# Sudaraka88/LDWeaver

Measured on AMD Instinct MI355X. Metric: MI SNP-pairs/sec, higher is better.
Workload: dtype i8

## Files before the change

### ldweaver_amd/csrc/ldw_apx.hip

```cpp
#include <algorithm>
#include <cmath>
#include <cstdlib>
#include <cstring>

#include "ldw_apx.h"
#include "ldw_dev.h"

using namespace ldw;

namespace ldw {

namespace {
constexpr int64_t APX_PROD_CAP = 12000;
struct ProdTable {
    std::vector<int32_t> val;
    std::vector<uint8_t> a, b;
    ProdTable() {
        std::vector<std::pair<int32_t, std::pair<uint8_t, uint8_t>>> all;
        for (int x = 0; x <= 127; ++x)
            for (int y = x; y <= 127; ++y) all.push_back({x * y, {(uint8_t)x, (uint8_t)y}});
        std::sort(all.begin(), all.end());
        for (auto &e : all)
            if (val.empty() || val.back() != e.first) {
                val.push_back(e.first);
// ... 824 lines not shown
    else if (tile == 33 && !P.fuse) {
        const int ntx = (P.RFpad + 95) / 96, nty = (P.RTpad + 95) / 96;
        if (P.fine) hipLaunchKernelGGL((gemm_apx_kernel<3, 3, true, 2>), dim3((unsigned)((ntx + 1) / 2), (unsigned)((nty + 1) / 2)), dim3(256), lds, st, P);
        else hipLaunchKernelGGL((gemm_apx_kernel<3, 3, false, 2>), dim3((unsigned)((ntx + 1) / 2), (unsigned)((nty + 1) / 2)), dim3(256), lds, st, P);
    }
    else if (tile == 224 && !P.fuse) {
        const int ntx = P.RFpad / 64, nty = P.RTpad / 64;
        if (P.fine) hipLaunchKernelGGL((gemm_apx_kernel<2, 2, true, 4>), dim3((unsigned)((ntx + 1) / 2), (unsigned)((nty + 1) / 2)), dim3(256), lds, st, P);
        else hipLaunchKernelGGL((gemm_apx_kernel<2, 2, false, 4>), dim3((unsigned)((ntx + 1) / 2), (unsigned)((nty + 1) / 2)), dim3(256), lds, st, P);
    }
    else if (tile == 24 && !P.fuse) LDW_APX_LAUNCH(2, 4)
    else if (tile == 32 && !P.fuse) {
        const int ntx = P.RFpad / 64, nty = (P.RTpad + 95) / 96;
        if (P.fine) hipLaunchKernelGGL((gemm_apx_kernel<3, 2, true, 3>), dim3((unsigned)((ntx + 1) / 2), (unsigned)((nty + 1) / 2)), dim3(256), lds, st, P);
        else hipLaunchKernelGGL((gemm_apx_kernel<3, 2, false, 3>), dim3((unsigned)((ntx + 1) / 2), (unsigned)((nty + 1) / 2)), dim3(256), lds, st, P);
    }
#endif
    else LDW_APX_LAUNCH(4, 2)
#undef LDW_APX_LAUNCH
    LDW_HIP(hipGetLastError());
    {
        const int tl = P.fuse ? 42 : tile;
        const int MTv = (P.fuse && P.skip_ctr) ? APX_MT : (tl == 22 || tl == 24 || tl == 224 ? 2 : (tl == 32 || tl == 33 ? 3 : 4)), NTv = tl == 24 ? 4 : (tl == 33 ? 3 : 2), TH = 32 * MTv, TWd = 32 * NTv;
        int64_t waves = 0;
        for (int ty = 0; ty * TH < P.RTpad; ++ty) {
            const int ntx = P.RFpad / TWd;
            if (!P.lower_only) waves += ntx;
            else for (int tx = 0; tx < ntx; ++tx) waves += (tx * TWd + TWd - 1 < ty * TH) ? 0 : 1;
        }
        c->gemm_stat[0] += 1;
        if (P.fuse) c->gemm_stat[5] += 1;
        c->gemm_stat[1] += 2.0 * (double)waves * TH * TWd * ((double)P.M2 * 128.0);
        if (P.fuse && P.skip_ctr) {
            c->apx_ops_per_wave = 2.0 * TH * TWd * ((double)P.M2 * 128.0);
            c->apx_waves_total += waves;
        }
    }
    return LDW_OK;
}

struct PairArgs {
    const uint64_t *Mbits;
    int64_t KW;
    int nwords, path, nseg;
    int seg_in_lds;
    const PopSeg *segs;
    const int32_t *wbeg, *row0;
    int32_t zero_row;
    int64_t *sums;
    EpiArgs A;
    unsigned long long *ghist;
};

template <int CA, int CB>
__device__ __forceinline__ void pair_sums_body(const PairArgs &P, int path, const int32_t *s_wbeg, const PopSeg *s_segs) {
    constexpr bool GENB = CA == 4 && CB == 4;
    const EpiArgs &A = P.A;
    const int sub = path * PAIR_SHARDS + (int)blockIdx.y;
    unsigned int n = A.pl_n[sub];
    n = n > A.pl_cap ? A.pl_cap : n;
    const int lane = threadIdx.x & 63;
    const PairEnt *list = A.pl_pairs + (int64_t)sub * A.pl_cap;
    constexpr int KW = 3, KS = 2;
    uint32_t smask[KW][KS];
    int64_t sV[KW][KS];
    bool more[KW];
#pragma unroll
    for (int k = 0; k < KW; ++k) {
        const int w = lane + 64 * k;
        int s0 = 0, s1 = 0;
        if (w < P.nwords) {
            s0 = s_wbeg[w] & 0x7FFFFFFF;
            s1 = s_wbeg[w + 1] & 0x7FFFFFFF;
        }
        more[k] = s1 - s0 > KS;
#pragma unroll
        for (int q = 0; q < KS; ++q) {
            const bool on = s0 + q < s1 && !more[k];
            smask[k][q] = on ? s_segs[s0 + q].mask : 0u;
            sV[k][q] = on ? s_segs[s0 + q].V : 0;
        }
    }
    for (unsigned int idx = blockIdx.x * 4u + (threadIdx.x >> 6); idx < n; idx += gridDim.x * 4u) {
        const PairEnt e = list[idx];
        const uint32_t era = (uint32_t)__builtin_amdgcn_readfirstlane((int)e.ra), erb = (uint32_t)__builtin_amdgcn_readfirstlane((int)e.rb);
        const int r0a = (int)(era & 0x1FFFFFFFu), na = (int)(era >> 29), r0b = (int)(erb & 0x1FFFFFFFu), nb = (int)(erb >> 29);
        const uint32_t *fr[CA], *tr[CB];
#pragma unroll
        for (int i = 0; i < CA; ++i) fr[i] = reinterpret_cast<const uint32_t *>(P.Mbits + (int64_t)(i < na ? r0a + i : P.zero_row) * P.KW);
#pragma unroll
        for (int j = 0; j < CB; ++j) tr[j] = reinterpret_cast<const uint32_t *>(P.Mbits + (int64_t)(j < nb ? r0b + j : P.zero_row) * P.KW);
        int64_t s[CB][CA];
#pragma unroll
        for (int j = 0; j < CB; ++j)
#pragma unroll
            for (int i = 0; i < CA; ++i) s[j][i] = 0;
        uint32_t f[KW][CA], tt[KW][CB];
#pragma unroll
        for (int k = 0; k < KW; ++k) {
            const int w = lane + 64 * k;
            const bool in = w < P.nwords;
#pragma unroll
            for (int i = 0; i < CA; ++i) f[k][i] = (in && (!GENB || i < na)) ? fr[i][w] : 0u;
#pragma unroll
            for (int j = 0; j < CB; ++j) tt[k][j] = (in && (!GENB || j < nb)) ? tr[j][w] : 0u;
        }
// ... 5 lines not shown
                for (int sg = s0; sg < s1; ++sg) {
                    const PopSeg seg = s_segs[sg];
#pragma unroll
                    for (int j = 0; j < CB; ++j)
#pragma unroll
                        for (int i = 0; i < CA; ++i)
                            if (!GENB || (i < na && j < nb)) s[j][i] += (int64_t)((uint64_t)__popc(f[k][i] & tt[k][j] & seg.mask) * (uint64_t)seg.V);
                }
            } else {
#pragma unroll
                for (int q2 = 0; q2 < KS; ++q2)
#pragma unroll
                    for (int j = 0; j < CB; ++j)
#pragma unroll
                        for (int i = 0; i < CA; ++i)
                            if (!GENB || (i < na && j < nb)) s[j][i] += (int64_t)((uint64_t)__popc(f[k][i] & tt[k][j] & smask[k][q2]) * (uint64_t)sV[k][q2]);
            }
        }
        for (int w = lane + 64 * KW; w < P.nwords; w += 64) {
            uint32_t f2[CA], t2[CB];
#pragma unroll
            for (int i = 0; i < CA; ++i) f2[i] = (!GENB || i < na) ? fr[i][w] : 0u;
#pragma unroll
            for (int j = 0; j < CB; ++j) t2[j] = (!GENB || j < nb) ? tr[j][w] : 0u;
            const int s0 = s_wbeg[w] & 0x7FFFFFFF, s1 = s_wbeg[w + 1] & 0x7FFFFFFF;
            for (int sg = s0; sg < s1; ++sg) {
                const PopSeg seg = s_segs[sg];
#pragma unroll
                for (int j = 0; j < CB; ++j)
#pragma unroll
                    for (int i = 0; i < CA; ++i)
                        if (!GENB || (i < na && j < nb)) s[j][i] += (int64_t)((uint64_t)__popc(f2[i] & t2[j] & seg.mask) * (uint64_t)seg.V);
            }
        }
#pragma unroll
        for (int j = 0; j < CB; ++j)
#pragma unroll
            for (int i = 0; i < CA; ++i) {
                int64_t v = s[j][i];
                if (!GENB || (i < na && j < nb)) {
#pragma unroll
                    for (int off = 32; off > 0; off >>= 1) v += __shfl_xor(v, off);
                }
                if (lane == 0) P.sums[((int64_t)sub * A.pl_cap + idx) * 16 + j * 4 + i] = v;
            }
    }
}

template <bool GEN>
__global__ __launch_bounds__(256) void k_pair_sums(PairArgs P) {
    extern __shared__ __attribute__((aligned(16))) uint8_t pop_smem[];
    int32_t *s_wbeg = reinterpret_cast<int32_t *>(pop_smem);
    PopSeg *s_segs = reinterpret_cast<PopSeg *>(pop_smem + (((size_t)P.nwords + 4) * 4 + 15) / 16 * 16);
    const int path = GEN ? 4 : (int)blockIdx.z;
    if (blockIdx.x * 4u >= P.A.pl_n[path * PAIR_SHARDS + (int)blockIdx.y]) return;
    if (P.seg_in_lds) {
        for (int i = threadIdx.x; i < P.nwords + 1; i += 256) s_wbeg[i] = P.wbeg[i];
        for (int i = threadIdx.x; i < P.nseg; i += 256) s_segs[i] = P.segs[i];
        __syncthreads();
    } else {
        s_wbeg = const_cast<int32_t *>(P.wbeg);
        s_segs = const_cast<PopSeg *>(P.segs);
    }
    if constexpr (GEN) {
        pair_sums_body<4, 4>(P, 4, s_wbeg, s_segs);
    } else {
        switch (path) {
            case 0: pair_sums_body<1, 1>(P, 0, s_wbeg, s_segs); break;
            case 1: pair_sums_body<2, 1>(P, 1, s_wbeg, s_segs); break;
            case 2: pair_sums_body<1, 2>(P, 2, s_wbeg, s_segs); break;
            default: pair_sums_body<2, 2>(P, 3, s_wbeg, s_segs); break;
        }
    }
}

template <int CA, int CB>
__device__ __forceinline__ void pair_sums_bits_body(const PairArgs &P, int path, const int64_t *sVT, int stride) {
    constexpr bool GENB = CA == 4 && CB == 4;
    const EpiArgs &A = P.A;
    const int sub = path * PAIR_SHARDS + (int)blockIdx.y;
    unsigned int n = A.pl_n[sub];
    n = n > A.pl_cap ? A.pl_cap : n;
    const int lane = threadIdx.x & 63;
    const PairEnt *list = A.pl_pairs + (int64_t)sub * A.pl_cap;
    for (unsigned int idx = blockIdx.x * 4u + (threadIdx.x >> 6); idx < n; idx += gridDim.x * 4u) {
        const PairEnt e = list[idx];
        const uint32_t era = (uint32_t)__builtin_amdgcn_readfirstlane((int)e.ra), erb = (uint32_t)__builtin_amdgcn_readfirstlane((int)e.rb);
        const int r0a = (int)(era & 0x1FFFFFFFu), na = (int)(era >> 29), r0b = (int)(erb & 0x1FFFFFFFu), nb = (int)(erb >> 29);
        const uint32_t *fr[CA], *tr[CB];
#pragma unroll
        for (int i = 0; i < CA; ++i) fr[i] = reinterpret_cast<const uint32_t *>(P.Mbits + (int64_t)(i < na ? r0a + i : P.zero_row) * P.KW);
#pragma unroll
        for (int j = 0; j < CB; ++j) tr[j] = reinterpret_cast<const uint32_t *>(P.Mbits + (int64_t)(j < nb ? r0b + j : P.zero_row) * P.KW);
        int64_t s[CB][CA];
#pragma unroll
        for (int j = 0; j < CB; ++j)
#pragma unroll
            for (int i = 0; i < CA; ++i) s[j][i] = 0;
        for (int w = lane; w < P.nwords; w += 64) {
            uint32_t f[CA], t[CB], uf = 0u, ut = 0u;
#pragma unroll
            for (int i = 0; i < CA; ++i) {
                f[i] = (!GENB || i < na) ? fr[i][w] : 0u;
                uf |= f[i];
            }
#pragma unroll
            for (int j = 0; j < CB; ++j) {
// ... 2 lines not shown
            }
            uint32_t u = uf & ut;
            while (u) {
                const int b = __builtin_ctz(u);
                u &= u - 1u;
                const int64_t v = sVT[b * stride + w];
#pragma unroll
                for (int j = 0; j < CB; ++j)
#pragma unroll
                    for (int i = 0; i < CA; ++i)
                        if (CA * CB == 1 || (((f[i] & t[j]) >> b) & 1u)) s[j][i] += v;
            }
        }
#pragma unroll
        for (int j = 0; j < CB; ++j)
#pragma unroll
            for (int i = 0; i < CA; ++i) {
                int64_t v = s[j][i];
                if (!GENB || (i < na && j < nb)) {
#pragma unroll
                    for (int off = 32; off > 0; off >>= 1) v += __shfl_xor(v, off);
                }
                if (lane == 0) P.sums[((int64_t)sub * A.pl_cap + idx) * 16 + j * 4 + i] = v;
            }
    }
}

template <bool GEN>
__global__ __launch_bounds__(256) void k_pair_sums_bits(PairArgs P, const int64_t *__restrict__ vpos, int stride) {
    extern __shared__ __attribute__((aligned(16))) uint8_t pop_smem[];
    int64_t *sVT = reinterpret_cast<int64_t *>(pop_smem);
    const int path = GEN ? 4 : (int)blockIdx.z;
    if (blockIdx.x * 4u >= P.A.pl_n[path * PAIR_SHARDS + (int)blockIdx.y]) return;
    for (int i = threadIdx.x; i < 32 * stride; i += 256) {
        const int b = i / stride, w = i - b * stride;
        sVT[i] = w < P.nwords ? vpos[32 * w + b] : 0;
    }
    __syncthreads();
    if constexpr (GEN) {
        pair_sums_bits_body<4, 4>(P, 4, sVT, stride);
    } else {
        switch (path) {
            case 0: pair_sums_bits_body<1, 1>(P, 0, sVT, stride); break;
            case 1: pair_sums_bits_body<2, 1>(P, 1, sVT, stride); break;
            case 2: pair_sums_bits_body<1, 2>(P, 2, sVT, stride); break;
            default: pair_sums_bits_body<2, 2>(P, 3, sVT, stride); break;
        }
    }
}

constexpr int PAIR_HWIN = 128;

template <int NA, int NB>
__device__ __forceinline__ void pair_mi_body(const PairArgs &P, int path, unsigned int *s_hist) {
    constexpr bool GEN = NA == 0;
    const EpiArgs &A = P.A;
    const EmitArgs &E = A.E;
    const int sub = path * PAIR_SHARDS + (int)blockIdx.y;
    unsigned int n = A.pl_n[sub];
    n = n > A.pl_cap ? A.pl_cap : n;
    const bool square = A.nf == A.nt;
    const PairEnt *list = A.pl_pairs + (int64_t)sub * A.pl_cap;
    const int lane = (int)(threadIdx.x & 63);
    for (unsigned int base = blockIdx.x * 256u + (threadIdx.x & ~63u); base < n; base += gridDim.x * 256u) {
        const unsigned int idx = base + (unsigned int)lane;
        bool valid = idx < n;
        uint32_t t = 0, q = 0;
        if (valid) {
            t = list[idx].t;
            q = list[idx].q;
        }
        const RowPack &RP = A.rowpack[t];
        valid = valid && RP.a_loc >= 0;
        bool cand = false;
        int bk = 0, seg = -1, a_loc = 0, b_loc = 0, sg = 0;
        double mi = 0.0;
        if (valid) {
            const RowSide R = RP.R;
            a_loc = RP.a_loc;
            const ColMeta M = A.colpack[q];
            b_loc = M.bl;
            sg = A.span ? M.ci.pad[0] : 0;
            const int64_t *sp = P.sums + ((int64_t)sub * A.pl_cap + idx) * 16;
            if constexpr (GEN) {
                mi = pair_mi<4, 4>(A, R, M, a_loc, b_loc, square, gacc_plain(sp, 1, 4));
            } else {
                mi = pair_mi_full<NA, NB>(A, R, M, a_loc, b_loc, square, gacc_plain(sp, 1, 4));
            }
            seg = pair_seg(a_loc, b_loc, E.lower_only);
            if (seg >= 0 && E.any_sr && col_is_sr(M.ci, a_loc)) {
                emit_pair_spec(E, M.ci, a_loc, b_loc, R.sa, M.sb, mi, P.ghist);
            } else if (seg >= 0 && E.do_lr && mi >= E.spec_lo) {
                bk = mi_bucket(mi);
                cand = bk >= E.spec_B;
            }
        }
        if (A.span) {
            for (int k = 0; k < A.span; ++k) {
                const bool mine = cand && sg == k;
                const unsigned long long mk = __ballot(mine);
                if (mk == 0ull) continue;
                const int leader = __builtin_ctzll(mk);
                unsigned long long pos = 0;
                if (lane == leader) pos = atomicAdd(A.sseg[k].n_cand, (unsigned long long)__popcll(mk));
                pos = __shfl(pos, leader);
                if (mine) {
                    pos += (unsigned long long)__popcll(mk & ((1ull << lane) - 1ull));
                    A.sseg[k].ckey[pos] = f64_key(mi);
                    A.sseg[k].cval[pos] = ((uint64_t)seg << 62) | ((uint64_t)a_loc + (uint64_t)b_loc * (uint64_t)E.nf);
                    const int w = bk - (E.spec_B > 0 ? E.spec_B : 0);
                    if (w < PAIR_HWIN) atomicAdd(&s_hist[k * PAIR_HWIN + w], 1u);
                    else atomicAdd(&A.sseg[k].ghist[bk], 1ull);
                }
            }
            continue;
        }
        const unsigned long long mk = __ballot(cand);
        if (mk == 0ull) continue;
        const int leader = __builtin_ctzll(mk);
        unsigned long long pos = 0;
        if (lane == leader) pos = atomicAdd(E.n_cand, (unsigned long long)__popcll(mk));
        pos = __shfl(pos, leader);
        if (cand) {
            pos += (unsigned long long)__popcll(mk & ((1ull << lane) - 1ull));
            E.ckey[pos] = f64_key(mi);
            E.cval[pos] = ((uint64_t)seg << 62) | ((uint64_t)a_loc + (uint64_t)b_loc * (uint64_t)E.nf);
            const int w = bk - (E.spec_B > 0 ? E.spec_B : 0);
            if (w < PAIR_HWIN) atomicAdd(&s_hist[w], 1u);
            else atomicAdd(&P.ghist[bk], 1ull);
        }
    }
}

__global__ __launch_bounds__(256) void k_pair_mi(PairArgs P) {
    __shared__ unsigned int s_hist[LDW_SPAN_MAX * PAIR_HWIN];
    for (int i = threadIdx.x; i < LDW_SPAN_MAX * PAIR_HWIN; i += 256) s_hist[i] = 0u;
    __syncthreads();
    switch (blockIdx.z) {
        case 0: pair_mi_body<1, 1>(P, 0, s_hist); break;
        case 1: pair_mi_body<2, 1>(P, 1, s_hist); break;
        case 2: pair_mi_body<1, 2>(P, 2, s_hist); break;
        case 3: pair_mi_body<2, 2>(P, 3, s_hist); break;
        default: pair_mi_body<0, 0>(P, 4, s_hist); break;
    }
    __syncthreads();
    const int hb0 = P.A.E.spec_B > 0 ? P.A.E.spec_B : 0;
    if (P.A.span) {
        for (int i = threadIdx.x; i < P.A.span * PAIR_HWIN; i += 256) {
            const int k = i / PAIR_HWIN, w = i - k * PAIR_HWIN;
            if (s_hist[i] != 0u && hb0 + w < NBINS) atomicAdd(&P.A.sseg[k].ghist[hb0 + w], (unsigned long long)s_hist[i]);
        }
        return;
    }
    if (threadIdx.x < PAIR_HWIN && s_hist[threadIdx.x] != 0u && hb0 + (int)threadIdx.x < NBINS)
        atomicAdd(&P.ghist[hb0 + threadIdx.x], (unsigned long long)s_hist[threadIdx.x]);
}

int launch_pairs_exact(ldw_ctx *c, const EpiArgs &A, unsigned long long *ghist, int64_t *sums, hipStream_t st) {
    PairArgs P;
    memset(&P, 0, sizeof(P));
    P.Mbits = c->Mbits.as<uint64_t>();
    P.KW = c->KW;
    P.nwords = (int)(c->KW * 2);
    P.nseg = c->n_pop_segs;
    P.segs = c->pop_segs.as<PopSeg>();
    P.wbeg = c->pop_wbeg.as<int32_t>();
    P.row0 = c->row0.as<int32_t>();
    P.zero_row = (int32_t)c->R;
    P.sums = sums;
    P.A = A;
    P.ghist = ghist;
    size_t lds = (((size_t)P.nwords + 4) * 4 + 15) / 16 * 16 + (size_t)P.nseg * sizeof(PopSeg);
    P.seg_in_lds = lds <= 60000 ? 1 : 0;
    if (!P.seg_in_lds) lds = 0;
    const int stride = (P.nwords + 31) / 32 * 32;
    const size_t lds_bits = (size_t)32 * stride * 8;
    const bool bits_off = getenv("LDW_NO_PAIR_BITS") != nullptr;
    const bool many_classes = !P.seg_in_lds || P.nseg >= 8 * P.nwords;
    if (many_classes && !bits_off && lds_bits <= 160 * 1024 && c->pop_vpos.p) {
        if (lds_bits > 64 * 1024 && !c->pair_bits_attr) {
            LDW_HIP(hipFuncSetAttribute(reinterpret_cast<const void *>(k_pair_sums_bits<false>), hipFuncAttributeMaxDynamicSharedMemorySize, 160 * 1024));
            LDW_HIP(hipFuncSetAttribute(reinterpret_cast<const void *>(k_pair_sums_bits<true>), hipFuncAttributeMaxDynamicSharedMemorySize, 160 * 1024));
            c->pair_bits_attr = true;
        }
        hipLaunchKernelGGL(k_pair_sums_bits<false>, dim3(256, PAIR_SHARDS, 4), dim3(256), lds_bits, st, P, c->pop_vpos.as<int64_t>(), stride);
        hipLaunchKernelGGL(k_pair_sums_bits<true>, dim3(256, PAIR_SHARDS, 1), dim3(256), lds_bits, st, P, c->pop_vpos.as<int64_t>(), stride);
    } else {
        static const unsigned gx_env = [] { const char *e = getenv("LDW_PAIR_GRID"); return e ? (unsigned)atoi(e) : 0u; }();
        hipLaunchKernelGGL(k_pair_sums<false>, dim3(gx_env ? gx_env : 512u, PAIR_SHARDS, 4), dim3(256), lds, st, P);
        hipLaunchKernelGGL(k_pair_sums<true>, dim3(gx_env ? gx_env : 1024u, PAIR_SHARDS, 1), dim3(256), lds, st, P);
    }
    hipLaunchKernelGGL(k_pair_mi, dim3(64, PAIR_SHARDS, PAIR_PATHS), dim3(256), 0, st, P);
    LDW_HIP(hipGetLastError());
    return LDW_OK;
}

}

namespace ldw {
void warm_apx() {
    hipFuncAttributes a;
    (void)hipFuncGetAttributes(&a, reinterpret_cast<const void *>(&k_pack_panel));
    (void)hipGetLastError();
}
}
```

### ldweaver_amd/csrc/ldw_internal.h

```cpp
#pragma once
#include <hip/hip_runtime.h>
#include <stdint.h>
#include <stdlib.h>
#include <string>
#include <atomic>
#include <memory>
#include <mutex>
#include <thread>
#include <vector>

#include "../../include/ldweaver_amd.h"

#define LDW_NSLOT 3

#ifdef LDW_EXPERIMENTS
#define LDW_HAS_EXPERIMENTS 1
#else
#define LDW_HAS_EXPERIMENTS 0
#endif

namespace ldw {

inline const char *exp_env(const char *name) {
#ifdef LDW_EXPERIMENTS
// ... 40 lines not shown
};
struct BlockTrace {
    int diag = 0, guess = -1, B_true = -1, margin = 0, path = 0 , missed = 0, probed = 0;
    long long n_cand = 0;
};

}

struct ldw_ctx {
    int device = 0;
    hipStream_t stream = nullptr;
    bool own_stream = true;
    hipEvent_t ev[6] = {nullptr, nullptr, nullptr, nullptr, nullptr, nullptr};
    double last_ms[4] = {0, 0, 0, 0};
    int engine = LDW_ENGINE_MFMA;

    int64_t L = 0, N = 0, Npad = 0;
    int64_t KW = 0;
    ldw::DevBuf states;
    ldw::DevBuf chars;
    int64_t cN = 0, cL = 0;
    void *fasta = nullptr;

    bool have_weights = false;
    int nlimbs = 5;
    int frac_bits = 0;
    double neff = 0;
    int64_t total_fixed = 0;
    ldw::DevBuf digits;
    ldw::DevBuf vfixed;
    std::vector<int64_t> h_vfixed;
    std::vector<int64_t> h_vfixed_hi;
    int64_t total_fixed_hi = 0;
    double lo_abs_sum = 0;
    int mixed = 1;

    std::vector<int32_t> h_seq_perm;
    ldw::DevBuf seq_perm;
    int path_mode = 0;
    int select_mode = 0;
    bool apx_ok = false;
    bool apx_fine = false;
    std::string apx_gate = "weights not set";
    ldw::DevBuf dig_a, dig_b;
    ldw::DevBuf apx_shift;
    int apx_e_last = 0;
    int apx_transitions = 0;
    double apx_lost_units = 0;
    double apx_delta = 0;
    std::vector<int64_t> h_vapx;
    ldw::DevBuf slot_papx;
    ldw::DevBuf pop_segs, pop_wbeg;
    ldw::DevBuf pop_vpos;
    bool pair_bits_attr = false;
    int n_pop_segs = 0, n_classes = 0;
    ldw::DevBuf panel[LDW_NSLOT][2];
    ldw::DevBuf Gapx[LDW_NSLOT];
    ldw::DevBuf tab11[2];
    double tab11_lo[2] = {0, 0};
    int tab11_cur[2] = {0, 0};
    int64_t tab11_builds = 0;
    float tab11_c = 0;
    int tab11_nb = 0;
    bool tab11_on = true;
    ldw::DevBuf pair_sums;
    ldw::DevBuf pairs[LDW_NSLOT];
    ldw::DevBuf sub_units[LDW_NSLOT], sub_packs[LDW_NSLOT], sub_bins[LDW_NSLOT], sub_live[LDW_NSLOT];
    ldw::DevBuf scr_live[LDW_NSLOT];
    ldw::DevBuf apx_bins[LDW_NSLOT], apx_clean[LDW_NSLOT];
    ldw::DevBuf apx_mini[LDW_NSLOT];
    ldw::DevBuf apx_units[LDW_NSLOT], apx_packs[LDW_NSLOT];
    int64_t apx_blocks = 0, apx_units_listed = 0, apx_pairs_listed = 0, probe_blocks = 0, generic_blocks = 0;
    bool prune = true;
    ldw::DevBuf apx_skip;
    double apx_ops_per_wave = 0;
    int64_t apx_waves_skipped = 0, apx_waves_total = 0;
    bool span_on = true;
    bool diag_split = false;
    bool span_corners = false;
    int span_max = 8;
    int64_t maybe_entries = 0;
    int64_t pair_list_overflows = 0, maybe_overflows = 0;
    bool maybe_off = false;
    int64_t span_items = 0, span_blocks = 0, span_fallbacks = 0;
    int64_t span_sr_subs = 0;
    bool early_sr = false;
    std::atomic<int64_t> sorted_blocks{0};
    std::mutex order_mtx;
    ldw::DevBuf snp_sup;
    double r_min = 0;
    struct OrderCache { std::vector<int32_t> idx, order; };
    std::vector<std::unique_ptr<OrderCache>> order_cache;

    bool have_meta = false;
    double g = 0;
    ldw::DevBuf r, uqe, POS, paint;
    std::vector<double> h_r;
    std::vector<int32_t> h_POS, h_paint;
    int32_t paint_min = 0, paint_max = 0;
    bool pos_sorted = true;
    double sr_total_dist = -1;
    int64_t sr_total = -1;
    uint64_t sr_share_key = 0;
    int64_t sr_share_rows = -1;

    bool rows_ready = false;
// ... 118 lines not shown
```

### ldweaver_amd/csrc/ldw_mi_items.inc

```
struct HostBlock {
    int64_t nf = 0, nt = 0, n_sr_blk = 0, n_lr_total = 0, blk_no = 0;
    int RFpad = 0, RTpad = 0, slot = 0;
    bool diag = false, fused = false, submitted = false;
    int nf_tiles = 0;
    int gen_t0 = 0, gen_q0 = 0;
    bool mixed = false;
    bool apx = false;
    bool generic = false;
    int guess = -1;
    LoHost lo;
    size_t o_cmax = 0, o_tbase = 0, o_tf = 0, o_band = 0, o_bandl = 0;
    int n_band = -1;
    size_t o_idx_f = 0, o_idx_t = 0, o_rl_f = 0, o_rl_t = 0, o_lrow_f = 0, o_lrow_t = 0, o_perm = 0, o_perm_t = 0, o_cols = 0, o_pos_f = 0,
           o_pos_t = 0, o_cls_f = 0, o_cls_t = 0, total = 0;
    DevPtrs D{};
    EmitArgs E{};
    int spec_B = -1;
    int span = 0;
    int32_t seg_start[LDW_SPAN_MAX] = {}, seg_nt[LDW_SPAN_MAX] = {};
    int64_t seg_lr_total[LDW_SPAN_MAX] = {};
    size_t cand_cap = 0;
    SpanSeg sseg[LDW_SPAN_MAX] = {};
    int pin_slot = -1;
    bool force_plain = false;
// ... 876 lines not shown
    const int32_t *ti = span.span_to.data() + span.seg_start[k];
    LDW_HIP(hipStreamSynchronize(c->stream));
    if (c->gemm_stream) LDW_HIP(hipStreamSynchronize(c->gemm_stream));
    if (int rc = prep_block(c, span.span_from.data(), span.nf, ti, span.seg_nt[k], p, span.slot, span.blk_no + k, hb, nullptr, LDW_NSLOT)) return rc;
    hb.force_plain = force_plain;
    ldw_mi_params q = *p;
    if (force_plain) q.keep_sr = 0;
    hb.sr_base = span.sr_base;
    for (int j = 0; j < k; ++j) hb.sr_base += span.seg_n_sr[j];
    hb.sr_base_fixed = true;
    p = &q;
    if (int rc = submit_a(c, hb, p, sl)) return rc;
    if (int rc = submit_b(c, hb, p, sl)) return rc;
    if (int rc = finish_block(c, hb, p, sl)) return rc;
    LDW_HIP(hipStreamSynchronize(c->stream));
    return LDW_OK;
}

int finish_span(ldw_ctx *c, HostBlock &hb, const ldw_mi_params *p, const SmallLayout &sl) {
    const int s = hb.slot;
    if (hb.span_alone) {
        for (int k = 0; k < hb.span; ++k)
            if (int rc = run_block_alone(c, hb, k, p, sl, false)) return rc;
        LDW_HIP(hipEventRecord(c->ev_done[s], c->stream));
        c->done_recorded[s] = true;
        return LDW_OK;
    }
    LDW_HIP(hipEventSynchronize(c->ev_pick[s]));
    ldw::PickOut picks[LDW_SPAN_MAX];
    for (int k = 0; k < hb.span; ++k) memcpy(&picks[k], static_cast<const char *>(c->pin_pick[s]) + (size_t)k * PICK_STRIDE, sizeof(ldw::PickOut));
    if (c->lrc_recorded) {
        LDW_HIP(hipEventSynchronize(c->ev_lrc));
        memcpy(&c->n_lr, c->pin_lrc, 8);
    }
    const char *d = stage_ptr(c, hb);
    if ((int64_t)c->trace.size() < hb.blk_no + hb.span) c->trace.resize((size_t)(hb.blk_no + hb.span));
    {
        static const bool trace_on = getenv("LDW_BLOCK_TRACE") != nullptr;
        if (trace_on && picks[0].n > 0 && !picks[0].spec_ok) {
            unsigned int pl[PAIR_PATHS * PAIR_SHARDS];
            LDW_HIP(hipMemcpy(pl, c->pairs[s].p, sizeof(pl), hipMemcpyDeviceToHost));
            fprintf(stderr, "[ldw span at block %lld] guess %d, %d segments, pair-list capacity %u, counters by path:", (long long)hb.blk_no, hb.guess, hb.span, pair_cap_for(hb.nf, hb.nt, hb.span));
            for (int pth = 0; pth < PAIR_PATHS; ++pth) {
                unsigned long long tot = 0, mx = 0;
                for (int sh2 = 0; sh2 < PAIR_SHARDS; ++sh2) {
                    tot += pl[pth * PAIR_SHARDS + sh2];
                    mx = std::max<unsigned long long>(mx, pl[pth * PAIR_SHARDS + sh2]);
                }
                fprintf(stderr, "  [%d] total %llu max %llu", pth, tot, mx);
            }
            fprintf(stderr, "\n");
        }
    }
    static const bool sel_fast_on = getenv("LDW_NO_FAST_SELECT") == nullptr && exp_env("LDW_NO_SPAN_SELECT") == nullptr;
    bool batched = sel_fast_on && c->select_mode == 0;
    long long m_max = 0, m_sum = 0;
    for (int k = 0; k < hb.span && batched; ++k) {
        const ldw::PickOut *hp = &picks[k];
        const uint64_t space = (uint64_t)hb.nf * (uint64_t)hb.seg_nt[k];
        const long long n_chunks = (long long)((2 * space + SEL_CHUNK_BITS - 1) / SEL_CHUNK_BITS) + 1, n_super = (n_chunks + SEL_SUPER - 1) / SEL_SUPER;
        batched = !(hp->n > 0 && !hp->spec_ok) && (long long)hp->n_cand <= SEL_MAX && n_super <= SEL_MAX_SUPER && (size_t)hp->n_cand <= hb.cand_cap;
        m_max = std::max<long long>(m_max, (long long)hp->n_cand);
        m_sum += (long long)hp->n_cand;
    }
    if (batched) {
        SelSpan S;
        memset(&S, 0, sizeof(S));
        SpanDoneArgs DA;
        memset(&DA, 0, sizeof(DA));
        S.n = hb.span;
        size_t w_off = 0, c_off = 0;
        size_t woff[LDW_SPAN_MAX], coff[LDW_SPAN_MAX];
        for (int k = 0; k < hb.span; ++k) {
            const uint64_t space = (uint64_t)hb.nf * (uint64_t)hb.seg_nt[k];
            const size_t n_words = (size_t)((2 * space + 31) / 32) + 1, n_chunks = (size_t)((2 * space + SEL_CHUNK_BITS - 1) / SEL_CHUNK_BITS) + 1;
            woff[k] = w_off;
            coff[k] = c_off;
            w_off += (n_words + 63) / 64 * 64;
            c_off += (n_chunks + 63) / 64 * 64;
            S.space[k] = space;
            S.n_super[k] = (int)((n_chunks + SEL_SUPER - 1) / SEL_SUPER);
        }
        if (w_off * 4 > c->sel_bitmap.cap || c_off * 4 > c->sel_chunks.cap || (size_t)LDW_SPAN_MAX * SEL_MAX_SUPER * 4 > c->sel_prefix.cap) {
            if (int rc = c->sel_bitmap.reserve(w_off * 4)) return rc;
            if (int rc = c->sel_chunks.reserve(c_off * 4)) return rc;
            if (int rc = c->sel_prefix.reserve((size_t)LDW_SPAN_MAX * SEL_MAX_SUPER * 4)) return rc;
            LDW_HIP(hipMemsetAsync(c->sel_bitmap.p, 0, c->sel_bitmap.cap, c->stream));
            LDW_HIP(hipMemsetAsync(c->sel_chunks.p, 0, c->sel_chunks.cap, c->stream));
            LDW_HIP(hipMemsetAsync(c->sel_prefix.p, 0, c->sel_prefix.cap, c->stream));
        }
        if (int rc = ensure_links_capacity(c, c->n_sr, c->n_lr + m_sum)) return rc;
        for (int k = 0; k < hb.span; ++k) {
            const ldw::PickOut *hp = &picks[k];
            if (hp->n > 0) update_guess(c, false, hp, false);
            ldw::BlockTrace &tr = c->trace[(size_t)hb.blk_no + k];
            tr = ldw::BlockTrace();
            tr.guess = hb.guess;
            tr.B_true = hp->B_true;
            tr.path = 4;
            tr.n_cand = (long long)hp->n_cand;
            S.ck[k] = hb.sseg[k].ckey;
            S.cv[k] = hb.sseg[k].cval;
            S.pick[k] = reinterpret_cast<ldw::PickOut *>(reinterpret_cast<char *>(sl.pick[s]) + (size_t)k * PICK_STRIDE);
            S.idx_t[k] = reinterpret_cast<const int32_t *>(d + hb.o_idx_t) + hb.seg_start[k];
            S.bitmap[k] = c->sel_bitmap.as<uint32_t>() + woff[k];
            S.chunks[k] = c->sel_chunks.as<uint32_t>() + coff[k];
// ... 127 lines not shown
```

Baseline: 163.1 billion.

## Add opt-in fused exact pair-sum and MI kernels with balanced run scheduling

Adds new kernels that split all pair lists into equal-size runs per wave, reuse loaded bit words across consecutive pairs sharing a row or column, and can fuse the popcount sums with the MI epilogue through LDS instead of global memory. These paths run only when LDW_PAIR_EXACT or LDW_PAIR_RUNS environment variables are set. By default the only behaviour change is that k_pair_sums now processes paths in reverse z order, and a pair-list statistics dump is added behind an env flag. The fused paths raise LDS use and register pressure in exchange for fewer global round trips and better load balance.

```diff
diff --git a/ldweaver_amd/csrc/ldw_apx.hip b/ldweaver_amd/csrc/ldw_apx.hip
--- a/ldweaver_amd/csrc/ldw_apx.hip
+++ b/ldweaver_amd/csrc/ldw_apx.hip
@@ -900,6 +900,149 @@
     unsigned long long *ghist;
 };
 
+constexpr int PAIR_KW = 3, PAIR_KS = 2;
+struct PairSegRegs {
+    uint32_t smask[PAIR_KW][PAIR_KS];
+    int64_t sV[PAIR_KW][PAIR_KS];
+    bool more[PAIR_KW];
+};
+__device__ __forceinline__ void pair_seg_regs(const PairArgs &P, const int32_t *s_wbeg, const PopSeg *s_segs, int lane, PairSegRegs &S) {
+#pragma unroll
+    for (int k = 0; k < PAIR_KW; ++k) {
+        const int w = lane + 64 * k;
+        int s0 = 0, s1 = 0;
+        if (w < P.nwords) {
+            s0 = s_wbeg[w] & 0x7FFFFFFF;
+            s1 = s_wbeg[w + 1] & 0x7FFFFFFF;
+        }
+        S.more[k] = s1 - s0 > PAIR_KS;
+#pragma unroll
+        for (int q = 0; q < PAIR_KS; ++q) {
+            const bool on = s0 + q < s1 && !S.more[k];
+            S.smask[k][q] = on ? s_segs[s0 + q].mask : 0u;
+            S.sV[k][q] = on ? s_segs[s0 + q].V : 0;
+        }
+    }
+}
+template <int CA, int CB>
+struct PairWords {
+    uint32_t f[PAIR_KW][CA], t[PAIR_KW][CB];
+};
+template <int CA, int CB>
+__device__ __forceinline__ const uint32_t *pair_row(const PairArgs &P, int r0, int n, int i) {
+    return reinterpret_cast<const uint32_t *>(P.Mbits + (int64_t)(i < n ? r0 + i : P.zero_row) * P.KW);
+}
+template <int CA, int CB, bool F, bool T>
+__device__ __forceinline__ void pair_load_words(const PairArgs &P, int lane, int r0a, int na, int r0b, int nb, PairWords<CA, CB> &W) {
+    constexpr bool GENB = CA == 4 && CB == 4;
+#pragma unroll
+    for (int k = 0; k < PAIR_KW; ++k) {
+        const int w = lane + 64 * k;
+        const bool in = w < P.nwords;
+        if constexpr (F) {
+#pragma unroll
+            for (int i = 0; i < CA; ++i) W.f[k][i] = (in && (!GENB || i < na)) ? pair_row<CA, CB>(P, r0a, na, i)[w] : 0u;
+        }
+        if constexpr (T) {
+#pragma unroll
+            for (int j = 0; j < CB; ++j) W.t[k][j] = (in && (!GENB || j < nb)) ? pair_row<CA, CB>(P, r0b, nb, j)[w] : 0u;
+        }
+    }
+}
+template <int CA, int CB>
+__device__ __forceinline__ void pair_lane_sums(const PairArgs &P, int lane, int r0a, int na, int r0b, int nb, const PairWords<CA, CB> &W,
+                                               const PairSegRegs &S, const int32_t *s_wbeg, const PopSeg *s_segs, int64_t (&s)[CB][CA]) {
+    constexpr bool GENB = CA == 4 && CB == 4;
+#pragma unroll
+    for (int j = 0; j < CB; ++j)
+#pragma unroll
+        for (int i = 0; i < CA; ++i) s[j][i] = 0;
+#pragma unroll
+    for (int k = 0; k < PAIR_KW; ++k) {
+        if (S.more[k]) {
+            const int w = lane + 64 * k;
+            const int s0 = s_wbeg[w] & 0x7FFFFFFF, s1 = s_wbeg[w + 1] & 0x7FFFFFFF;
+            for (int sg = s0; sg < s1; ++sg) {
+                const PopSeg seg = s_segs[sg];
+#pragma unroll
+                for (int j = 0; j < CB; ++j)
+#pragma unroll
+                    for (int i = 0; i < CA; ++i)
+                        if (!GENB || (i < na && j < nb)) s[j][i] += (int64_t)((uint64_t)__popc(W.f[k][i] & W.t[k][j] & seg.mask) * (uint64_t)seg.V);
+            }
+        } else {
+#pragma unroll
+            for (int q2 = 0; q2 < PAIR_KS; ++q2)
+#pragma unroll
+                for (int j = 0; j < CB; ++j)
+#pragma unroll
+                    for (int i = 0; i < CA; ++i)
+                        if (!GENB || (i < na && j < nb)) s[j][i] += (int64_t)((uint64_t)__popc(W.f[k][i] & W.t[k][j] & S.smask[k][q2]) * (uint64_t)S.sV[k][q2]);
+        }
+    }
+    for (int w = lane + 64 * PAIR_KW; w < P.nwords; w += 64) {
+        uint32_t f2[CA], t2[CB];
+#pragma unroll
+        for (int i = 0; i < CA; ++i) f2[i] = (!GENB || i < na) ? pair_row<CA, CB>(P, r0a, na, i)[w] : 0u;
+#pragma unroll
+        for (int j = 0; j < CB; ++j) t2[j] = (!GENB || j < nb) ? pair_row<CA, CB>(P, r0b, nb, j)[w] : 0u;
+        const int s0 = s_wbeg[w] & 0x7FFFFFFF, s1 = s_wbeg[w + 1] & 0x7FFFFFFF;
+        for (int sg = s0; sg < s1; ++sg) {
+            const PopSeg seg = s_segs[sg];
+#pragma unroll
+            for (int j = 0; j < CB; ++j)
+#pragma unroll
+                for (int i = 0; i < CA; ++i)
+                    if (!GENB || (i < na && j < nb)) s[j][i] += (int64_t)((uint64_t)__popc(f2[i] & t2[j] & seg.mask) * (uint64_t)seg.V);
+        }
+    }
+}
+template <int CA, int CB>
+__device__ __forceinline__ void pair_reduce_store(int lane, int na, int nb, int64_t (&s)[CB][CA], int64_t *out, int so) {
+    constexpr bool GENB = CA == 4 && CB == 4;
+#pragma unroll
+    for (int j = 0; j < CB; ++j)
+#pragma unroll
+        for (int i = 0; i < CA; ++i) {
+            int64_t v = s[j][i];
+            if (!GENB || (i < na && j < nb)) {
+#pragma unroll
+                for (int off = 32; off > 0; off >>= 1) v += __shfl_xor(v, off);
+            }
+            if (lane == 0) out[j * so + i] = v;
+        }
+}
+
+template <int CA, int CB>
+__device__ __forceinline__ void pair_reduce_scatter_store(int lane, int64_t (&s)[CB][CA], int64_t *out, int so) {
+    constexpr int M = CA * CB, LM = M == 4 ? 2 : (M == 2 ? 1 : 0);
+    static_assert(M == 1 || M == 2 || M == 4, "straight-line shapes only");
+    int64_t v[M];
+#pragma unroll
+    for (int j = 0; j < CB; ++j)
+#pragma unroll
+        for (int i = 0; i < CA; ++i) v[j * CA + i] = s[j][i];
+#pragma unroll
+    for (int st = 0, h = M / 2; st < LM; ++st, h /= 2) {
+        const int off = 32 >> st;
+        const bool up = (lane & off) != 0;
+#pragma unroll
+        for (int k = 0; k < M / 2; ++k) {
+            if (k < h) {
+                const int64_t keep = up ? v[k + h] : v[k], send = up ? v[k] : v[k + h];
+                v[k] = keep + __shfl_xor(send, off);
+            }
+        }
+    }
+    int64_t x = v[0];
+#pragma unroll
+    for (int off = 32 >> LM; off > 0; off >>= 1) x += __shfl_xor(x, off);
+    if ((lane & ((64 >> LM) - 1)) == 0) {
+        const int m = lane >> (6 - LM), j = m / CA, i = m - j * CA;
+        out[j * so + i] = x;
+    }
+}
+
 template <int CA, int CB>
 __device__ __forceinline__ void pair_sums_body(const PairArgs &P, int path, const int32_t *s_wbeg, const PopSeg *s_segs) {
     constexpr bool GENB = CA == 4 && CB == 4;
@@ -1011,7 +1154,7 @@
     extern __shared__ __attribute__((aligned(16))) uint8_t pop_smem[];
     int32_t *s_wbeg = reinterpret_cast<int32_t *>(pop_smem);
     PopSeg *s_segs = reinterpret_cast<PopSeg *>(pop_smem + (((size_t)P.nwords + 4) * 4 + 15) / 16 * 16);
-    const int path = GEN ? 4 : (int)blockIdx.z;
+    const int path = GEN ? 4 : 3 - (int)blockIdx.z;
     if (blockIdx.x * 4u >= P.A.pl_n[path * PAIR_SHARDS + (int)blockIdx.y]) return;
     if (P.seg_in_lds) {
         for (int i = threadIdx.x; i < P.nwords + 1; i += 256) s_wbeg[i] = P.wbeg[i];
@@ -1120,19 +1263,14 @@
 constexpr int PAIR_HWIN = 128;
 
 template <int NA, int NB>
-__device__ __forceinline__ void pair_mi_body(const PairArgs &P, int path, unsigned int *s_hist) {
+__device__ __forceinline__ void pair_mi_emit(const PairArgs &P, const PairEnt *list, unsigned int idx, bool valid, const int64_t *sp, int sj,
+                                             unsigned int *s_hist) {
     constexpr bool GEN = NA == 0;
     const EpiArgs &A = P.A;
     const EmitArgs &E = A.E;
-    const int sub = path * PAIR_SHARDS + (int)blockIdx.y;
-    unsigned int n = A.pl_n[sub];
-    n = n > A.pl_cap ? A.pl_cap : n;
     const bool square = A.nf == A.nt;
-    const PairEnt *list = A.pl_pairs + (int64_t)sub * A.pl_cap;
     const int lane = (int)(threadIdx.x & 63);
-    for (unsigned int base = blockIdx.x * 256u + (threadIdx.x & ~63u); base < n; base += gridDim.x * 256u) {
-        const unsigned int idx = base + (unsigned int)lane;
-        bool valid = idx < n;
+    {
         uint32_t t = 0, q = 0;
         if (valid) {
             t = list[idx].t;
@@ -1149,11 +1287,10 @@
             const ColMeta M = A.colpack[q];
             b_loc = M.bl;
             sg = A.span ? M.ci.pad[0] : 0;
-            const int64_t *sp = P.sums + ((int64_t)sub * A.pl_cap + idx) * 16;
             if constexpr (GEN) {
-                mi = pair_mi<4, 4>(A, R, M, a_loc, b_loc, square, gacc_plain(sp, 1, 4));
+                mi = pair_mi<4, 4>(A, R, M, a_loc, b_loc, square, gacc_plain(sp, 1, sj));
             } else {
-                mi = pair_mi_full<NA, NB>(A, R, M, a_loc, b_loc, square, gacc_plain(sp, 1, 4));
+                mi = pair_mi_full<NA, NB>(A, R, M, a_loc, b_loc, square, gacc_plain(sp, 1, sj));
             }
             seg = pair_seg(a_loc, b_loc, E.lower_only);
             if (seg >= 0 && E.any_sr && col_is_sr(M.ci, a_loc)) {
@@ -1181,10 +1318,10 @@
                     else atomicAdd(&A.sseg[k].ghist[bk], 1ull);
                 }
             }
-            continue;
+            return;
         }
         const unsigned long long mk = __ballot(cand);
-        if (mk == 0ull) continue;
+        if (mk == 0ull) return;
         const int leader = __builtin_ctzll(mk);
         unsigned long long pos = 0;
         if (lane == leader) pos = atomicAdd(E.n_cand, (unsigned long long)__popcll(mk));
@@ -1200,11 +1337,38 @@
     }
 }
 
+template <int NA, int NB>
+__device__ __forceinline__ void pair_mi_body(const PairArgs &P, int path, unsigned int *s_hist) {
+    const EpiArgs &A = P.A;
+    const int sub = path * PAIR_SHARDS + (int)blockIdx.y;
+    unsigned int n = A.pl_n[sub];
+    n = n > A.pl_cap ? A.pl_cap : n;
+    const PairEnt *list = A.pl_pairs + (int64_t)sub * A.pl_cap;
+    const int lane = (int)(threadIdx.x & 63);
+    for (unsigned int base = blockIdx.x * 256u + (threadIdx.x & ~63u); base < n; base += gridDim.x * 256u) {
+        const unsigned int idx = base + (unsigned int)lane;
+        pair_mi_emit<NA, NB>(P, list, idx, idx < n, P.sums + ((int64_t)sub * A.pl_cap + idx) * 16, 4, s_hist);
+    }
+}
+
+__device__ __forceinline__ void pair_hist_flush(const PairArgs &P, const unsigned int *s_hist) {
+    const int hb0 = P.A.E.spec_B > 0 ? P.A.E.spec_B : 0;
+    if (P.A.span) {
+        for (int i = threadIdx.x; i < P.A.span * PAIR_HWIN; i += 256) {
+            const int k = i / PAIR_HWIN, w = i - k * PAIR_HWIN;
+            if (s_hist[i] != 0u && hb0 + w < NBINS) atomicAdd(&P.A.sseg[k].ghist[hb0 + w], (unsigned long long)s_hist[i]);
+        }
+        return;
+    }
+    if (threadIdx.x < PAIR_HWIN && s_hist[threadIdx.x] != 0u && hb0 + (int)threadIdx.x < NBINS)
+        atomicAdd(&P.ghist[hb0 + threadIdx.x], (unsigned long long)s_hist[threadIdx.x]);
+}
+
 __global__ __launch_bounds__(256) void k_pair_mi(PairArgs P) {
     __shared__ unsigned int s_hist[LDW_SPAN_MAX * PAIR_HWIN];
     for (int i = threadIdx.x; i < LDW_SPAN_MAX * PAIR_HWIN; i += 256) s_hist[i] = 0u;
     __syncthreads();
-    switch (blockIdx.z) {
+    switch ((int)blockIdx.z + P.path) {
         case 0: pair_mi_body<1, 1>(P, 0, s_hist); break;
         case 1: pair_mi_body<2, 1>(P, 1, s_hist); break;
         case 2: pair_mi_body<1, 2>(P, 2, s_hist); break;
@@ -1212,16 +1376,163 @@
         default: pair_mi_body<0, 0>(P, 4, s_hist); break;
     }
     __syncthreads();
-    const int hb0 = P.A.E.spec_B > 0 ? P.A.E.spec_B : 0;
-    if (P.A.span) {
-        for (int i = threadIdx.x; i < P.A.span * PAIR_HWIN; i += 256) {
-            const int k = i / PAIR_HWIN, w = i - k * PAIR_HWIN;
-            if (s_hist[i] != 0u && hb0 + w < NBINS) atomicAdd(&P.A.sseg[k].ghist[hb0 + w], (unsigned long long)s_hist[i]);
-        }
-        return;
-    }
-    if (threadIdx.x < PAIR_HWIN && s_hist[threadIdx.x] != 0u && hb0 + (int)threadIdx.x < NBINS)
-        atomicAdd(&P.ghist[hb0 + threadIdx.x], (unsigned long long)s_hist[threadIdx.x]);
+    pair_hist_flush(P, s_hist);
+}
+
+constexpr int PX_BATCH = 64;
+template <bool GEN> constexpr int px_slot() { return GEN ? 16 : 4; }
+
+template <int CA, int CB, int NA, int NB, bool FUSE>
+__device__ __forceinline__ void pair_exact_run(const PairArgs &P, int sub, unsigned int c0, unsigned int c1, const int32_t *s_wbeg, const PopSeg *s_segs,
+                                               const PairSegRegs &S, int64_t *s_sum, int so, unsigned int *s_hist) {
+    const EpiArgs &A = P.A;
+    const int lane = (int)(threadIdx.x & 63);
+    const PairEnt *list = A.pl_pairs + (int64_t)sub * A.pl_cap;
+    for (unsigned int b0 = c0; b0 < c1; b0 += PX_BATCH) {
+        const int nb_pairs = (int)(c1 - b0 < (unsigned int)PX_BATCH ? c1 - b0 : (unsigned int)PX_BATCH);
+        uint32_t my_ra = 0u, my_rb = 0u;
+        if (lane < nb_pairs) {
+            my_ra = list[b0 + lane].ra;
+            my_rb = list[b0 + lane].rb;
+        }
+        uint32_t era = (uint32_t)__builtin_amdgcn_readlane((int)my_ra, 0), erb = (uint32_t)__builtin_amdgcn_readlane((int)my_rb, 0);
+        PairWords<CA, CB> W;
+        pair_load_words<CA, CB, true, true>(P, lane, (int)(era & 0x1FFFFFFFu), (int)(era >> 29), (int)(erb & 0x1FFFFFFFu), (int)(erb >> 29), W);
+        for (int k = 0; k < nb_pairs; ++k) {
+            const int r0a = (int)(era & 0x1FFFFFFFu), na = (int)(era >> 29), r0b = (int)(erb & 0x1FFFFFFFu), nb = (int)(erb >> 29);
+            PairWords<CA, CB> Wn = W;
+            uint32_t nra = era, nrb = erb;
+            if (k + 1 < nb_pairs) {
+                nra = (uint32_t)__builtin_amdgcn_readlane((int)my_ra, k + 1);
+                nrb = (uint32_t)__builtin_amdgcn_readlane((int)my_rb, k + 1);
+                const int n0a = (int)(nra & 0x1FFFFFFFu), nna = (int)(nra >> 29), n0b = (int)(nrb & 0x1FFFFFFFu), nnb = (int)(nrb >> 29);
+                if (nra != era && nrb != erb) pair_load_words<CA, CB, true, true>(P, lane, n0a, nna, n0b, nnb, Wn);
+                else if (nra != era) pair_load_words<CA, CB, true, false>(P, lane, n0a, nna, n0b, nnb, Wn);
+                else if (nrb != erb) pair_load_words<CA, CB, false, true>(P, lane, n0a, nna, n0b, nnb, Wn);
+            }
+            int64_t s[CB][CA];
+            pair_lane_sums<CA, CB>(P, lane, r0a, na, r0b, nb, W, S, s_wbeg, s_segs, s);
+            int64_t *out = FUSE ? s_sum + k * so : P.sums + ((int64_t)sub * A.pl_cap + b0 + (unsigned int)k) * 16;
+            constexpr int SJ = FUSE ? CA : 4;
+            if constexpr (CA == 4 && CB == 4) pair_reduce_store<CA, CB>(lane, na, nb, s, out, SJ);
+            else pair_reduce_scatter_store<CA, CB>(lane, s, out, SJ);
+            W = Wn;
+            era = nra;
+            erb = nrb;
+        }
+        if constexpr (!FUSE) continue;
+        __builtin_amdgcn_fence(__ATOMIC_RELEASE, "wavefront");
+        __builtin_amdgcn_wave_barrier();
+        __builtin_amdgcn_fence(__ATOMIC_ACQUIRE, "wavefront");
+        pair_mi_emit<NA, NB>(P, list, b0 + (unsigned int)lane, lane < nb_pairs, s_sum + lane * so, CA, s_hist);
+        __builtin_amdgcn_fence(__ATOMIC_RELEASE, "wavefront");
+        __builtin_amdgcn_wave_barrier();
+        __builtin_amdgcn_fence(__ATOMIC_ACQUIRE, "wavefront");
+    }
+}
+
+constexpr int PX_NL_MAX = 4 * PAIR_SHARDS;
+__host__ __device__ constexpr size_t px_lds_fixed(bool gen, bool fuse) {
+    return (fuse ? (size_t)LDW_SPAN_MAX * PAIR_HWIN * 4 + (size_t)4 * PX_BATCH * (gen ? 16 : 4) * 8 : 0) + (size_t)(2 * PX_NL_MAX + 4) * 4;
+}
+
+template <bool GEN, bool FUSE>
+__device__ __forceinline__ void pair_runs_body(const PairArgs &P, uint8_t *pop_smem) {
+    constexpr int SO = FUSE ? px_slot<GEN>() : 0;
+    constexpr int HW = FUSE ? LDW_SPAN_MAX * PAIR_HWIN : 0;
+    constexpr int NL = GEN ? PAIR_SHARDS : 4 * PAIR_SHARDS;
+    constexpr int P0 = GEN ? 4 : 0;
+    unsigned int *s_hist = reinterpret_cast<unsigned int *>(pop_smem);
+    int64_t *s_sum = reinterpret_cast<int64_t *>(pop_smem + (size_t)HW * 4);
+    unsigned int *s_n = reinterpret_cast<unsigned int *>(pop_smem + (size_t)HW * 4 + (size_t)4 * PX_BATCH * SO * 8);
+    unsigned int *s_pre = s_n + PX_NL_MAX;
+    int32_t *s_wbeg = reinterpret_cast<int32_t *>(pop_smem + px_lds_fixed(GEN, FUSE));
+    PopSeg *s_segs = reinterpret_cast<PopSeg *>(pop_smem + px_lds_fixed(GEN, FUSE) + (((size_t)P.nwords + 4) * 4 + 15) / 16 * 16);
+    for (int i = threadIdx.x; i < HW; i += 256) s_hist[i] = 0u;
+    if (threadIdx.x < NL) {
+        const unsigned int n = P.A.pl_n[P0 * PAIR_SHARDS + threadIdx.x];
+        s_n[threadIdx.x] = n > P.A.pl_cap ? P.A.pl_cap : n;
+    }
+    if (P.seg_in_lds) {
+        for (int i = threadIdx.x; i < P.nwords + 1; i += 256) s_wbeg[i] = P.wbeg[i];
+        for (int i = threadIdx.x; i < P.nseg; i += 256) s_segs[i] = P.segs[i];
+    } else {
+        s_wbeg = const_cast<int32_t *>(P.wbeg);
+        s_segs = const_cast<PopSeg *>(P.segs);
+    }
+    __syncthreads();
+    if (threadIdx.x == 0) {
+        unsigned long long tot = 0;
+        for (int l = 0; l < NL; ++l) tot += s_n[l];
+        const unsigned long long waves = (unsigned long long)gridDim.x * 4ull;
+        const unsigned int C = (unsigned int)(tot > waves ? (tot + waves - 1) / waves : 1ull);
+        unsigned int r = 0;
+        for (int l = 0; l < NL; ++l) {
+            s_pre[l] = r;
+            r += (s_n[l] + C - 1) / C;
+        }
+        s_pre[NL] = r;
+        s_pre[NL + 1] = C;
+    }
+    __syncthreads();
+    const int lane = (int)(threadIdx.x & 63), wv = (int)(threadIdx.x >> 6);
+    PairSegRegs S;
+    pair_seg_regs(P, s_wbeg, s_segs, lane, S);
+    const unsigned int runs = s_pre[NL], C = s_pre[NL + 1];
+    int64_t *my_sum = s_sum + (size_t)wv * PX_BATCH * SO;
+    int l = 0;
+    for (unsigned int g = blockIdx.x * 4u + (unsigned int)wv; g < runs; g += gridDim.x * 4u) {
+        while (s_pre[l + 1] <= g) ++l;
+        const unsigned int c0 = (g - s_pre[l]) * C, c1 = c0 + C < s_n[l] ? c0 + C : s_n[l];
+        const int sub = P0 * PAIR_SHARDS + l;
+        if constexpr (GEN) {
+            pair_exact_run<4, 4, 0, 0, FUSE>(P, sub, c0, c1, s_wbeg, s_segs, S, my_sum, SO, s_hist);
+        } else {
+            switch (l / PAIR_SHARDS) {
+                case 0: pair_exact_run<1, 1, 1, 1, FUSE>(P, sub, c0, c1, s_wbeg, s_segs, S, my_sum, SO, s_hist); break;
+                case 1: pair_exact_run<2, 1, 2, 1, FUSE>(P, sub, c0, c1, s_wbeg, s_segs, S, my_sum, SO, s_hist); break;
+                case 2: pair_exact_run<1, 2, 1, 2, FUSE>(P, sub, c0, c1, s_wbeg, s_segs, S, my_sum, SO, s_hist); break;
+                default: pair_exact_run<2, 2, 2, 2, FUSE>(P, sub, c0, c1, s_wbeg, s_segs, S, my_sum, SO, s_hist); break;
+            }
+        }
+    }
+    if constexpr (FUSE) {
+        __syncthreads();
+        pair_hist_flush(P, s_hist);
+    }
+}
+
+template <bool GEN>
+__global__ __launch_bounds__(256) void k_pair_exact(PairArgs P) {
+    extern __shared__ __attribute__((aligned(16))) uint8_t pop_smem[];
+    pair_runs_body<GEN, true>(P, pop_smem);
+}
+
+template <bool GEN>
+__global__ __launch_bounds__(256) void k_pair_runs(PairArgs P) {
+    extern __shared__ __attribute__((aligned(16))) uint8_t pop_smem[];
+    pair_runs_body<GEN, false>(P, pop_smem);
+}
+
+template <bool GEN, bool FUSE>
+static int pair_exact_grid(size_t lds) {
+    static int cus = 0;
+    if (!cus) {
+        int dev = 0;
+        (void)hipGetDevice(&dev);
+        if (hipDeviceGetAttribute(&cus, hipDeviceAttributeMultiprocessorCount, dev) != hipSuccess || cus <= 0) cus = 256;
+    }
+    static size_t last_lds = ~(size_t)0;
+    static int per_cu = 0;
+    if (last_lds != lds) {
+        const void *k = FUSE ? reinterpret_cast<const void *>(k_pair_exact<GEN>) : reinterpret_cast<const void *>(k_pair_runs<GEN>);
+        int b = 0;
+        if (hipOccupancyMaxActiveBlocksPerMultiprocessor(&b, k, 256, lds) != hipSuccess || b <= 0) b = 1;
+        (void)hipGetLastError();
+        per_cu = b;
+        last_lds = lds;
+    }
+    return cus * per_cu;
 }
 
 int launch_pairs_exact(ldw_ctx *c, const EpiArgs &A, unsigned long long *ghist, int64_t *sums, hipStream_t st) {
@@ -1255,8 +1566,30 @@
         hipLaunchKernelGGL(k_pair_sums_bits<true>, dim3(256, PAIR_SHARDS, 1), dim3(256), lds_bits, st, P, c->pop_vpos.as<int64_t>(), stride);
     } else {
         static const unsigned gx_env = [] { const char *e = getenv("LDW_PAIR_GRID"); return e ? (unsigned)atoi(e) : 0u; }();
-        hipLaunchKernelGGL(k_pair_sums<false>, dim3(gx_env ? gx_env : 512u, PAIR_SHARDS, 4), dim3(256), lds, st, P);
-        hipLaunchKernelGGL(k_pair_sums<true>, dim3(gx_env ? gx_env : 1024u, PAIR_SHARDS, 1), dim3(256), lds, st, P);
+        if (getenv("LDW_PAIR_EXACT") != nullptr) {
+            const size_t ldsx = lds + px_lds_fixed(false, true), ldsg = lds + px_lds_fixed(true, true);
+            if (ldsg > 64 * 1024 && !c->pair_exact_attr) {
+                LDW_HIP(hipFuncSetAttribute(reinterpret_cast<const void *>(k_pair_exact<false>), hipFuncAttributeMaxDynamicSharedMemorySize, 160 * 1024));
+                LDW_HIP(hipFuncSetAttribute(reinterpret_cast<const void *>(k_pair_exact<true>), hipFuncAttributeMaxDynamicSharedMemorySize, 160 * 1024));
+                c->pair_exact_attr = true;
+            }
+            hipLaunchKernelGGL(k_pair_exact<false>, dim3(gx_env ? gx_env : (unsigned)pair_exact_grid<false, true>(ldsx)), dim3(256), ldsx, st, P);
+            if (getenv("LDW_PAIR_EXACT_GEN") != nullptr) {
+                hipLaunchKernelGGL(k_pair_exact<true>, dim3(gx_env ? gx_env : (unsigned)pair_exact_grid<true, true>(ldsg)), dim3(256), ldsg, st, P);
+                LDW_HIP(hipGetLastError());
+                return LDW_OK;
+            }
+            hipLaunchKernelGGL(k_pair_sums<true>, dim3(gx_env ? gx_env : 1024u, PAIR_SHARDS, 1), dim3(256), lds, st, P);
+            P.path = 4;
+            hipLaunchKernelGGL(k_pair_mi, dim3(64, PAIR_SHARDS, 1), dim3(256), 0, st, P);
+            LDW_HIP(hipGetLastError());
+            return LDW_OK;
+        }
+        const size_t ldsr = lds + px_lds_fixed(false, false);
+        if (getenv("LDW_PAIR_RUNS") == nullptr) hipLaunchKernelGGL(k_pair_sums<false>, dim3(gx_env ? gx_env : 512u, PAIR_SHARDS, 4), dim3(256), lds, st, P);
+        else hipLaunchKernelGGL(k_pair_runs<false>, dim3(gx_env ? gx_env : (unsigned)pair_exact_grid<false, false>(ldsr)), dim3(256), ldsr, st, P);
+        if (getenv("LDW_PAIR_RUNS_GEN") != nullptr) hipLaunchKernelGGL(k_pair_runs<true>, dim3(gx_env ? gx_env : (unsigned)pair_exact_grid<true, false>(ldsr)), dim3(256), ldsr, st, P);
+        else hipLaunchKernelGGL(k_pair_sums<true>, dim3(gx_env ? gx_env : 1024u, PAIR_SHARDS, 1), dim3(256), lds, st, P);
     }
     hipLaunchKernelGGL(k_pair_mi, dim3(64, PAIR_SHARDS, PAIR_PATHS), dim3(256), 0, st, P);
     LDW_HIP(hipGetLastError());
diff --git a/ldweaver_amd/csrc/ldw_internal.h b/ldweaver_amd/csrc/ldw_internal.h
--- a/ldweaver_amd/csrc/ldw_internal.h
+++ b/ldweaver_amd/csrc/ldw_internal.h
@@ -116,6 +116,7 @@
     ldw::DevBuf slot_papx;
     ldw::DevBuf pop_segs, pop_wbeg;
     ldw::DevBuf pop_vpos;
+    bool pair_exact_attr = false;
     bool pair_bits_attr = false;
     int n_pop_segs = 0, n_classes = 0;
     ldw::DevBuf panel[LDW_NSLOT][2];
diff --git a/ldweaver_amd/csrc/ldw_mi_items.inc b/ldweaver_amd/csrc/ldw_mi_items.inc
--- a/ldweaver_amd/csrc/ldw_mi_items.inc
+++ b/ldweaver_amd/csrc/ldw_mi_items.inc
@@ -952,6 +952,32 @@
             fprintf(stderr, "\n");
         }
     }
+    {
+        static const bool pl_stats = getenv("LDW_PAIR_LIST_STATS") != nullptr;
+        if (pl_stats && c->pairs[s].p) {
+            const uint32_t cap = pair_cap_for(hb.nf, hb.nt, hb.span);
+            unsigned int pl[PAIR_PATHS * PAIR_SHARDS];
+            LDW_HIP(hipMemcpy(pl, c->pairs[s].p, sizeof(pl), hipMemcpyDeviceToHost));
+            std::vector<PairEnt> ent;
+            unsigned long long tot = 0, mx = 0, same_a = 0, same_b = 0, steps = 0, by_path[PAIR_PATHS] = {0, 0, 0, 0, 0};
+            for (int l = 0; l < PAIR_PATHS * PAIR_SHARDS; ++l) {
+                const unsigned int n = std::min<unsigned int>(pl[l], cap);
+                tot += n;
+                by_path[l / PAIR_SHARDS] += n;
+                mx = std::max<unsigned long long>(mx, n);
+                if (n < 2) continue;
+                ent.resize(n);
+                LDW_HIP(hipMemcpy(ent.data(), c->pairs[s].as<char>() + 256 + (size_t)l * cap * sizeof(PairEnt), (size_t)n * sizeof(PairEnt), hipMemcpyDeviceToHost));
+                for (unsigned int i = 1; i < n; ++i) {
+                    same_a += ent[i].ra == ent[i - 1].ra;
+                    same_b += ent[i].rb == ent[i - 1].rb;
+                }
+                steps += n - 1;
+            }
+            fprintf(stderr, "[ldw pair lists] block %lld span %d: pairs %llu (by path %llu %llu %llu %llu %llu), largest list %llu, consecutive entries sharing the row SNP %llu / column SNP %llu of %llu\n",
+                    (long long)hb.blk_no, hb.span, tot, by_path[0], by_path[1], by_path[2], by_path[3], by_path[4], mx, same_a, same_b, steps);
+        }
+    }
     static const bool sel_fast_on = getenv("LDW_NO_FAST_SELECT") == nullptr && exp_env("LDW_NO_SPAN_SELECT") == nullptr;
     bool batched = sel_fast_on && c->select_mode == 0;
     long long m_max = 0, m_sum = 0;
```

Measured after the change: 164.8 billion, median of 6. No clear change (+1.1%).
